# JuliaGenAI/ColBERT.jl

Measured on AMD Instinct MI355X. Metric: queries/sec, top-1000 on 1M-passage corpus, higher is better.
Workload: dtype f32

## Files before the change

colbert.jl_amd/csrc/approx_kernels.hpp:

```cpp
#pragma once
#include <hip/hip_fp16.h>

#include <algorithm>

#include "common.hpp"
#include "search_kernels.hpp"

namespace clb {

typedef __bf16 bf16x8 __attribute__((ext_vector_type(8)));
typedef uint32_t u32x4 __attribute__((ext_vector_type(4)));
typedef uint32_t u32x4_a4 __attribute__((ext_vector_type(4), aligned(4)));
typedef float f32x4_a4 __attribute__((ext_vector_type(4), aligned(4)));

constexpr float kEpsSafety = 1.25f;

inline bool approx_supported(int dim, int nbits) { return dim == kDim && nbits == 2; }
inline size_t approx_cells_bytes(int64_t B, int64_t K, int64_t ) { return (size_t)B * K * 16 * 4 + 2048; }

__device__ __forceinline__ uint32_t f32_to_bf16_rne(float f) {
    const uint32_t u = __float_as_uint(f);
    return (u + 0x7fffu + ((u >> 16) & 1u)) >> 16;
}
__device__ __forceinline__ uint32_t pack_bf16(float lo, float hi) {
// ... 739 lines not shown
        }
        const float v[4] = {__uint_as_float(lo.x), __uint_as_float(lo.z), __uint_as_float(hi.x), __uint_as_float(hi.z)};
        const int id[4] = {(int)lo.y, (int)lo.w, (int)hi.y, (int)hi.w};
#pragma unroll
        for (int e = 0; e < 4; ++e) {
            const bool take = id[e] != 0x7fffffff && v[e] >= thr;
            const unsigned long long m = __builtin_amdgcn_ballot_w64(take);
            if (m == 0) break;
            const int pos = total + __popcll(m & ((1ull << lane) - 1ull));
            if (take && pos < kTopRefineCap) cand[pos] = ValIdx{v[e], id[e]};
            total += __popcll(m);
        }
    }
    __syncthreads();
    const bool overflow = total > kTopRefineCap || last_max >= thr;
    float tv[2] = {kNegInf, kNegInf};
    int ti[2] = {0x7fffffff, 0x7fffffff};
    if (!overflow) {
        for (int g0 = 0; g0 < total; g0 += kTopRefine) {
        const int grp = g0 + (lane >> 4), rr = lane & 15;
        const int gid = grp < total ? cand[grp].i : 0;
        const int id = (gid >> 1) * 32 + (rr & 3) + 8 * (rr >> 2) + 4 * (gid & 1);
        if (grp < total && id < K) {
            const float4* c4 = reinterpret_cast<const float4*>(C + (size_t)id * kDim);
            float4 cr[32];
#pragma unroll
            for (int m = 0; m < 32; ++m) cr[m] = c4[m];
            float a = 0.f;
#pragma unroll
            for (int m = 0; m < 32; ++m) {
                a = fmaf(cr[m].x, qs[4 * m], a);
                a = fmaf(cr[m].y, qs[4 * m + 1], a);
                a = fmaf(cr[m].z, qs[4 * m + 2], a);
                a = fmaf(cr[m].w, qs[4 * m + 3], a);
            }
            topn_insert<2>(tv, ti, a, id);
        }
        }
    } else {
        for (int c = lane; c < K; c += 64) {
            const float* cr = C + (size_t)c * kDim;
            float a = 0.f;
            for (int d = 0; d < kDim; ++d) a = fmaf(cr[d], qs[d], a);
            topn_insert<2>(tv, ti, a, c);
        }
        if (lane == 0) atomicAdd(&redo_flag[b], 1);
    }
#pragma unroll
    for (int o = 32; o > 0; o >>= 1) {
        const float v0 = __shfl_xor(tv[0], o, 64), v1 = __shfl_xor(tv[1], o, 64);
        const int i0 = __shfl_xor(ti[0], o, 64), i1 = __shfl_xor(ti[1], o, 64);
        topn_insert<2>(tv, ti, v0, i0);
        topn_insert<2>(tv, ti, v1, i1);
    }
    if (lane == 0) {
        sel[((size_t)b * 32 + t) * 2] = ti[0];
        sel[((size_t)b * 32 + t) * 2 + 1] = ti[1] == 0x7fffffff ? ti[0] : ti[1];
    }
}

static __global__ __launch_bounds__(256) void cells_to_half_kernel(const float* __restrict__ cells,
                                                                  uint32_t* __restrict__ cells16, int K) {
    const int b = blockIdx.y;
    const float* src = cells + (size_t)b * K * 32;
    uint32_t* dst = cells16 + (size_t)b * K * 16;
    const int64_t total = (int64_t)K * 16;
    for (int64_t i = (int64_t)blockIdx.x * 256 + threadIdx.x; i < total; i += (int64_t)gridDim.x * 256) {
        const int64_t c = i >> 4;
        const int t = (int)(i & 15);
        const float lo = src[c * 32 + 2 * t], hi = src[c * 32 + 2 * t + 1];
        const __half2 h = __floats2half2_rn(lo, hi);
        dst[i] = *reinterpret_cast<const uint32_t*>(&h);
    }
}

typedef _Float16 f16x8 __attribute__((ext_vector_type(8)));
typedef float f32x2 __attribute__((ext_vector_type(2)));

struct StepTag {
    int j;
    int rows;
    int last;
    int base;
};

constexpr int kStepRows = 32;

__device__ __forceinline__ uint32_t f32_to_f16_floor(float x) {
    const __half hr = __float2half_rn(x);
    uint32_t bits = *reinterpret_cast<const uint16_t*>(&hr);
    if (__half2float(hr) > x) bits = (bits & 0x8000u) ? bits + 1u : (bits == 0u ? 0x8001u : bits - 1u);
    return bits;
}

template <int N>
__device__ __forceinline__ uint32_t lut_offset(uint32_t R, uint32_t lane8) {
    return __builtin_amdgcn_perm(R, lane8, 0x0c0c0000u | ((4u + N) << 8));
}

#define CLB_DPP_F(V, CTRL) __builtin_bit_cast(float, __builtin_amdgcn_update_dpp(0, __builtin_bit_cast(int, (V)), (CTRL), 0xf, 0xf, true))
__device__ __forceinline__ float sum_lanes_0_31(float s) {
    s += CLB_DPP_F(s, 0xB1);
    s += CLB_DPP_F(s, 0x4E);
    s += CLB_DPP_F(s, 0x141);
    s += CLB_DPP_F(s, 0x140);
    const float below = __builtin_bit_cast(float, __builtin_amdgcn_update_dpp(0, __builtin_bit_cast(int, s), 0x142, 0xa, 0xf, false));
    return s + below;
}
__device__ __forceinline__ float max_lane_halves(float m) { return fmaxf(m, __shfl_xor(m, 32, 64)); }

#ifndef CLB_APPROX_WAVES
#define CLB_APPROX_WAVES 12
#endif
#ifdef CLB_APPROX_SPLIT_LUT
constexpr bool kSplitLut = true;
#else
constexpr bool kSplitLut = false;
#endif
#if defined(CLB_APPROX_PRIO) && CLB_APPROX_PRIO
#define CLB_APPROX_PRIO_UP __builtin_amdgcn_s_setprio(CLB_APPROX_PRIO);
#define CLB_APPROX_PRIO_DOWN __builtin_amdgcn_s_setprio(0);
#else
#define CLB_APPROX_PRIO_UP
#define CLB_APPROX_PRIO_DOWN
#endif
#ifndef CLB_APPROX_MINOCC
#define CLB_APPROX_MINOCC (CLB_APPROX_WAVES / 4)
#endif
constexpr int kApproxThreads = 64 * CLB_APPROX_WAVES;
constexpr int kApproxLdsLut = 256 * 256;

template <bool ROWS, int ABL = 0, int GL = 0, int PIPE = 0, bool CELL8 = false>
static __global__ __launch_bounds__(kApproxThreads, CLB_APPROX_MINOCC) void score_approx32_kernel(
    const float* __restrict__ weights, const uint32_t* __restrict__ codeinv, const uint8_t* __restrict__ residuals,
    int cbits, float inv_lo, float inv_step, const float* __restrict__ Q, const uint32_t* __restrict__ cells16,
    const uint2* __restrict__ cand_hdr, const int* __restrict__ ncand, float* __restrict__ scores, int K, int T,
    int B, size_t cand_cap, uint16_t* __restrict__ tokmax, const int* __restrict__ list,
    const int* __restrict__ nlist, const float* __restrict__ eps_pair, unsigned long long* __restrict__ rowmask,
    const float4* __restrict__ tscale = nullptr) {
    const uint32_t cmask = (1u << cbits) - 1u;
    const int lane = threadIdx.x & 63;
    const int r = lane & 31, h = lane >> 5;
    const int x = blockIdx.x & 7;
    const int wg = blockIdx.x >> 3;
    const int wg_per_group = gridDim.x >> 3;
    const int wave = __builtin_amdgcn_readfirstlane(threadIdx.x >> 6);
    __shared__ __attribute__((aligned(16))) unsigned char lut_s[kApproxLdsLut];
    __shared__ __attribute__((aligned(16))) float invx[kApproxThreads / 64][2 * kStepRows];
    static_assert(GL == 0 || ABL == 0, "the ablation variants exist for the VGPR gather only");
    static_assert(!CELL8 || ABL == 0, "the ablation variants exist for the fp16 score rows only");
    constexpr int kSlotBytes = CELL8 ? 1024 : 2048;
    constexpr int kRingBytes = 3 * kSlotBytes;
    static_assert(GL == 0 || CLB_APPROX_WAVES <= 12, "the 3-slot ring of the LDS-DMA form fits 160 KB of LDS up to 12 waves");
    __shared__ __attribute__((aligned(16))) unsigned char ring_s[GL ? (kApproxThreads / 64) * kRingBytes : 16];
    constexpr int kStageBytes = 16 * 64 + 64;
    __shared__ __attribute__((aligned(16))) unsigned char stage_s[ROWS ? 16 : (kApproxThreads / 64) * kStageBytes];
    unsigned char* mystage = stage_s + (ROWS ? 0 : wave * kStageBytes);
    for (int i = threadIdx.x; i < 256 * 32; i += kApproxThreads) {
        const int v = i >> 5;
        *reinterpret_cast<uint2*>(lut_s + (size_t)i * 8) =
            make_uint2(pack_f16(weights[v & 3], weights[(v >> 2) & 3]), pack_f16(weights[(v >> 4) & 3], weights[(v >> 6) & 3]));
    }
    __syncthreads();
    const char* lut = reinterpret_cast<const char*>(lut_s);
    float* myinv = invx[wave];
    const uint32_t lane8 = 8u * (uint32_t)r;
    unsigned char* myring = ring_s + (GL ? wave * kRingBytes : 0);
    const uint32_t ring_lds = (uint32_t)(uintptr_t)(__attribute__((address_space(3))) unsigned char*)myring;
    const uint32_t gl_poff = 16u * (((uint32_t)lane - (((uint32_t)lane >> 4) & 3u)) & 3u);
    const int gl_src0 = (int)((uint32_t)lane & ~3u);
    const int gl_src1 = gl_src0 + 64;
    const uint32_t gl_rot = ((uint32_t)r >> 2) & 3u;
    const uint32_t gl_x0 = (uint32_t)r * 64u + 16u * (((uint32_t)h + gl_rot) & 3u);
    const uint32_t gl_x1 = (uint32_t)r * 64u + 16u * (((uint32_t)h + 2u + gl_rot) & 3u);
    const int gl8_src = (int)(((uint32_t)lane >> 1) << 2);
    const uint32_t gl8_poff = 16u * (((uint32_t)lane ^ ((uint32_t)lane >> 4)) & 1u);
    const uint32_t gl8_x = (uint32_t)r * 32u + 16u * (((uint32_t)h ^ ((uint32_t)r >> 3)) & 1u);

    f16x8 sel1, sel2;
#pragma unroll
    for (int j = 0; j < 8; ++j) {
        sel1[j] = (r == (CELL8 ? 16 * h + j : 8 * h + j)) ? (_Float16)1.0f : (_Float16)0.0f;
        sel2[j] = (r == (CELL8 ? 16 * h + 8 + j : 16 + 8 * h + j)) ? (_Float16)1.0f : (_Float16)0.0f;
    }

    int b_first, b_step, sub, nsub;
    if (B >= 8) { b_first = x; b_step = 8; sub = 0; nsub = 1; }
    else { b_first = x % B; b_step = B * 8 ; sub = x / B; nsub = (8 - b_first + B - 1) / B; }
    const bool grid2d = gridDim.y > 1;
    const int wg_count = grid2d ? (int)gridDim.x : wg_per_group;
    const int wg_index = grid2d ? (int)blockIdx.x : wg;
    if (grid2d) { b_first = blockIdx.y; b_step = B; sub = 0; nsub = 1; }

    for (int b = b_first; b < B; b += b_step) {
        u32x4 qb[8];
        const float4 ts = CELL8 ? tscale[(size_t)b * 32 + r] : make_float4(1.f, 1.f, 0.f, 0.f);
        const float stp = ts.x;
        const float acc_init = CELL8 ? ts.z - 1024.0f : 0.f;
        {
            const float* qrow = Q + ((size_t)b * T + (r < T ? r : T - 1)) * kDim + 64 * h;
#pragma unroll
            for (int s = 0; s < 8; ++s) {
                float4 lo = *reinterpret_cast<const float4*>(qrow + 8 * s);
                float4 hi = *reinterpret_cast<const float4*>(qrow + 8 * s + 4);
                if (r >= T) { lo = make_float4(0.f, 0.f, 0.f, 0.f); hi = lo; }
                if (CELL8) {
                    lo.x *= ts.y; lo.y *= ts.y; lo.z *= ts.y; lo.w *= ts.y;
                    hi.x *= ts.y; hi.y *= ts.y; hi.z *= ts.y; hi.w *= ts.y;
                }
                qb[s] = u32x4{pack_f16(lo.x, lo.y), pack_f16(lo.z, lo.w), pack_f16(hi.x, hi.y), pack_f16(hi.z, hi.w)};
            }
        }
        const uint2* hdr = cand_hdr + (size_t)b * cand_cap;
        const char* c16 = reinterpret_cast<const char*>(cells16 + (size_t)b * K * (CELL8 ? 8 : 16));
        const uint32_t h16 = 16u * (uint32_t)h;
        float* out = scores + (size_t)b * cand_cap;
        uint16_t* tmax = tokmax + (size_t)b * cand_cap * 32 + r;
        const int* lst = ROWS ? list + (size_t)b * cand_cap : nullptr;
        unsigned long long* rmask = ROWS ? rowmask + (size_t)b * cand_cap * 4 : nullptr;
        const float window = ROWS ? 2.f * eps_pair[b] : 0.f;
        const int n = ROWS ? nlist[b] : ncand[b];
        const int n_waves = wg_count * (kApproxThreads / 64) * nsub;
        const int my_wave = (sub * wg_count + wg_index) * (kApproxThreads / 64) + wave;
        const int per_wave = (n + n_waves - 1) / n_waves;
        const int j_first = min(n, my_wave * per_wave), j_end = min(n, j_first + per_wave);
        unsigned long long wm0 = 0, wm1 = 0, wm2 = 0, wm3 = 0;

        for (int j0 = j_first; j0 < j_end; j0 += 64) {
        const int jl = j0 + lane;
        int slot_l = jl < j_end ? jl : j0;
        if (ROWS) slot_l = lst[slot_l];
        const uint2 hv = hdr[slot_l];
        const int nd = j_end - j0 < 64 ? j_end - j0 : 64;
        int it_k = 0;
        uint32_t it_off = __builtin_amdgcn_readlane(hv.x, 0);
        int it_len = (int)__builtin_amdgcn_readlane(hv.y, 0);
        int it_slot = __builtin_amdgcn_readlane(slot_l, 0);
        int it_base = 0;
        const uint32_t abl_stride = ABL == 11 ? ((uint32_t)__builtin_amdgcn_readlane(hv.x, nd - 1) - it_off) / (uint32_t)nd : 0u;
        if (ABL == 11) it_len = 82;
        const uint32_t abl_bound = ABL == 11 ? (uint32_t)__builtin_amdgcn_readlane(hv.x, nd - 1) : 0u;

#define CLB_STAGE_A(RB, CV, PM, TAG)                                                                    \
    {                                                                                                       \
        const bool live = it_k < nd;                                                                        \
        const uint32_t e0 = live ? (ABL == 11 ? min(it_off + (uint32_t)it_base, abl_bound) : it_off + (uint32_t)it_base) : 0u; \
        const int left = live ? it_len - it_base : kStepRows;                                               \
        const int rows = left < kStepRows ? left : kStepRows;                                               \
        if (ROWS) PM = tmax[(size_t)(live ? it_slot : 0) * 32];    \
        const uint32_t rr = min((uint32_t)r, (uint32_t)(rows - 1));    \
         \
        const uint8_t* rbase_ = residuals + (size_t)e0 * 32;                                                \
        const uint32_t* cbase_ = codeinv + (size_t)e0;                                                      \
        const uint32_t roff_ = rr * 32u + h16;                                                              \
         \
         \
        if (ABL == 3 || ABL == 7) RB = u32x4{e0 * 2654435761u + rr, e0 ^ h16, e0 + 77u * rr, e0 * 40503u};  \
        else if (ABL == 4) RB = *reinterpret_cast<const u32x4*>(rbase_ + roff_);                            \
        else RB = __builtin_nontemporal_load(reinterpret_cast<const u32x4*>(rbase_ + roff_));               \
        if (ABL == 7) CV = (e0 * 97u + rr) & 131071u;                                                       \
        else if (ABL == 4) CV = cbase_[rr];                                                                 \
        else CV = __builtin_nontemporal_load(cbase_ + rr);                    \
        TAG.j = live ? j0 + it_k : -1;                                                                      \
        TAG.rows = rows;                                                                                    \
        TAG.last = left <= kStepRows ? (it_k + 1 >= nd ? 3 : 1) : 0;                                        \
        TAG.base = it_base;                                                                                 \
        it_base += kStepRows;                                                                               \
        if (ABL == 11) {         \
            if (TAG.last) { it_k += 1; it_off += abl_stride; it_base = 0; }                                 \
        } else                                                                                              \
        if (TAG.last) {                                                                                     \
            it_k += 1;                                                                                      \
            const int kk = it_k < 64 ? it_k : 63;                                                           \
            it_off = __builtin_amdgcn_readlane(hv.x, kk);                                                   \
            it_len = (int)__builtin_amdgcn_readlane(hv.y, kk);                                              \
            it_slot = __builtin_amdgcn_readlane(slot_l, kk);                                                \
            it_base = 0;                                                                                    \
        }                                                                                                   \
    }
#define CLB_STAGE_G(CV, X0, X1, SLOT)                                                                       \
    if (GL && CELL8) {                                                                                      \
        const uint32_t ca_ = (uint32_t)__builtin_amdgcn_ds_bpermute(gl8_src, (int)CV) & cmask;              \
        asm volatile("s_mov_b32 m0, %1\n\tglobal_load_lds_dwordx4 %0, off"                                  \
                     :: "v"(c16 + ((ca_ << 5) + gl8_poff)), "s"(ring_lds + (SLOT) * 1024u) : "memory");     \
    } else if (GL) {                                                                                        \
        const uint32_t ca_ = (uint32_t)__builtin_amdgcn_ds_bpermute(gl_src0, (int)CV) & cmask;              \
        const uint32_t cb_ = (uint32_t)__builtin_amdgcn_ds_bpermute(gl_src1, (int)CV) & cmask;              \
         \
        asm volatile("s_mov_b32 m0, %2\n\tglobal_load_lds_dwordx4 %0, off\n\t"                            \
                     "s_add_u32 m0, m0, 0x400\n\tglobal_load_lds_dwordx4 %1, off"                          \
                     :: "v"(c16 + ((ca_ << 6) + gl_poff)), "v"(c16 + ((cb_ << 6) + gl_poff)),               \
                        "s"(ring_lds + (SLOT) * 2048u) : "memory", "scc");                                   \
    } else {                                                                                                \
        const char* row_ = CELL8 ? c16 + (((CV & cmask) << 5) + h16)                                        \
                                 : c16 + (((ABL == 2 ? (CV & 1023u) : (CV & cmask)) << 6) + h16);           \
        if (ABL == 1 || ABL == 7) { X0 = u32x4{CV, CV, CV, CV}; X1 = X0; }                                  \
        else if (CELL8) X0 = *reinterpret_cast<const u32x4*>(row_);       \
        else {                                                                                              \
        X0 = *reinterpret_cast<const u32x4*>(row_);                                                         \
        X1 = *reinterpret_cast<const u32x4*>(row_ + 32);                                                    \
        }                                                                                                   \
    }
#define CLB_LUT(W, N) (*reinterpret_cast<const uint2*>(lut + lut_offset<N>(W, lane8)))
#define CLB_STAGE_CM(RB, CV, X0, X1, SLOT, ACC, INVB)                                                       \
    {                                                                                                       \
        if (GL && CELL8) {                                                                                  \
             \
            asm volatile("s_waitcnt vmcnt(3)" ::: "memory");                                                \
            X0 = *reinterpret_cast<const u32x4*>(myring + (SLOT) * 1024 + gl8_x);                           \
        } else if (GL) {                                                                                    \
             \
            asm volatile("s_waitcnt vmcnt(4)" ::: "memory");                                                \
            X0 = *reinterpret_cast<const u32x4*>(myring + (SLOT) * 2048 + gl_x0);                           \
            X1 = *reinterpret_cast<const u32x4*>(myring + (SLOT) * 2048 + gl_x1);                           \
        }                                                                                                   \
         \
        __builtin_amdgcn_wave_barrier();                                                                    \
        myinv[(INVB) * kStepRows + r] = fmaf((float)(CV >> cbits), inv_step, inv_lo);                                            \
        __builtin_amdgcn_wave_barrier();                                                                    \
         \
         \
         \
        uint2 tl[16];                                                                                       \
        if (ABL != 5) {                                                                                     \
            tl[0] = CLB_LUT(RB[0], 0); tl[1] = CLB_LUT(RB[0], 1); tl[2] = CLB_LUT(RB[0], 2); tl[3] = CLB_LUT(RB[0], 3);     \
            tl[4] = CLB_LUT(RB[1], 0); tl[5] = CLB_LUT(RB[1], 1); tl[6] = CLB_LUT(RB[1], 2); tl[7] = CLB_LUT(RB[1], 3);     \
            if (!kSplitLut) {                                                                               \
            tl[8] = CLB_LUT(RB[2], 0); tl[9] = CLB_LUT(RB[2], 1); tl[10] = CLB_LUT(RB[2], 2); tl[11] = CLB_LUT(RB[2], 3);   \
            tl[12] = CLB_LUT(RB[3], 0); tl[13] = CLB_LUT(RB[3], 1); tl[14] = CLB_LUT(RB[3], 2); tl[15] = CLB_LUT(RB[3], 3); \
            }                                                                                               \
        }                                                                                                   \
        __builtin_amdgcn_sched_barrier(0);                                                                  \
        CLB_APPROX_PRIO_UP                                                                                  \
        _Pragma("unroll") for (int i = 0; i < 16; ++i) ACC[i] = acc_init;                                   \
        if (CELL8) {                     \
            const u32x4 raw_ = X0;                                                                          \
            X0 = u32x4{__builtin_amdgcn_perm(0x64646464u, raw_[0], 0x04010400u), __builtin_amdgcn_perm(0x64646464u, raw_[0], 0x04030402u), \
                       __builtin_amdgcn_perm(0x64646464u, raw_[1], 0x04010400u), __builtin_amdgcn_perm(0x64646464u, raw_[1], 0x04030402u)}; \
            X1 = u32x4{__builtin_amdgcn_perm(0x64646464u, raw_[2], 0x04010400u), __builtin_amdgcn_perm(0x64646464u, raw_[2], 0x04030402u), \
                       __builtin_amdgcn_perm(0x64646464u, raw_[3], 0x04010400u), __builtin_amdgcn_perm(0x64646464u, raw_[3], 0x04030402u)}; \
        }                                                                                                   \
        ACC = __builtin_amdgcn_mfma_f32_32x32x16_f16(__builtin_bit_cast(f16x8, X0), sel1, ACC, 0, 0, 0);    \
        ACC = __builtin_amdgcn_mfma_f32_32x32x16_f16(__builtin_bit_cast(f16x8, X1), sel2, ACC, 0, 0, 0);    \
        if (ABL == 5) { ACC[0] += __uint_as_float(RB[0] ^ RB[1]); ACC[1] += __uint_as_float(RB[2] ^ RB[3]); } \
        else {                                                                                              \
            _Pragma("unroll") for (int s_ = 0; s_ < 8; ++s_) {                                              \
                if (kSplitLut && s_ == 4) {       \
                    __builtin_amdgcn_sched_barrier(0);                                                      \
                    tl[0] = CLB_LUT(RB[2], 0); tl[1] = CLB_LUT(RB[2], 1); tl[2] = CLB_LUT(RB[2], 2); tl[3] = CLB_LUT(RB[2], 3);   \
                    tl[4] = CLB_LUT(RB[3], 0); tl[5] = CLB_LUT(RB[3], 1); tl[6] = CLB_LUT(RB[3], 2); tl[7] = CLB_LUT(RB[3], 3);   \
                    __builtin_amdgcn_sched_barrier(0);                                                      \
                }                                                                                           \
                const int ti_ = kSplitLut ? 2 * (s_ & 3) : 2 * s_;                                          \
                ACC = __builtin_amdgcn_mfma_f32_32x32x16_f16(                                               \
                    __builtin_bit_cast(f16x8, u32x4{tl[ti_].x, tl[ti_].y, tl[ti_ + 1].x, tl[ti_ + 1].y}),   \
                    __builtin_bit_cast(f16x8, qb[s_]), ACC, 0, 0, 0);                                       \
            }                                                                                               \
        }                                                                                                   \
        CLB_APPROX_PRIO_DOWN                                                                                \
    }
#define CLB_STAGE_E(ACC, INVB, PM, TAG)                                                                     \
    {                                                                                                       \
        f32x4 iq[4];                                                                                        \
        _Pragma("unroll") for (int q = 0; q < 4; ++q)                                                       \
            iq[q] = *reinterpret_cast<const f32x4*>(myinv + (INVB) * kStepRows + 8 * q + 4 * h);                                 \
         \
         \
         \
        float v[16];                                                                                        \
        if (ABL != 6) { _Pragma("unroll") for (int i = 0; i < 16; ++i) { v[i] = ACC[i] * iq[i >> 2][i & 3]; asm volatile("" : "+v"(v[i])); } } \
        else                                                                                                \
        _Pragma("unroll") for (int i = 0; i < 16; i += 2) {     \
            const f32x2 p_ = f32x2{ACC[i], ACC[i + 1]} * f32x2{iq[i >> 2][i & 3], iq[i >> 2][(i & 3) + 1]}; \
            v[i] = p_[0]; v[i + 1] = p_[1];                                                                 \
        }                                                                                                   \
        if (ROWS) {                                                                                         \
            const __half pmh = *reinterpret_cast<const __half*>(&PM);                                       \
            const float lo = r < T ? __half2float(pmh) - window : __builtin_inff();    \
             \
             \
             \
            uint32_t lm = 0;                                                                                \
            _Pragma("unroll") for (int i = 0; i < 16; ++i) lm |= !((CELL8 ? v[i] * stp : v[i]) < lo) ? (1u << i) : 0u; \
            lm |= (uint32_t)__builtin_amdgcn_update_dpp(0, (int)lm, 0xB1, 0xf, 0xf, true);         \
            lm |= (uint32_t)__builtin_amdgcn_update_dpp(0, (int)lm, 0x4E, 0xf, 0xf, true);         \
            lm |= (uint32_t)__builtin_amdgcn_update_dpp(0, (int)lm, 0x141, 0xf, 0xf, true);    \
            lm |= (uint32_t)__builtin_amdgcn_update_dpp(0, (int)lm, 0x140, 0xf, 0xf, true);      \
            const uint32_t m0_ = __builtin_amdgcn_readlane(lm, 0) | __builtin_amdgcn_readlane(lm, 16);      \
            const uint32_t m1_ = __builtin_amdgcn_readlane(lm, 32) | __builtin_amdgcn_readlane(lm, 48);     \
             \
            uint32_t bits = ((m0_ & 0xFu) | ((m0_ & 0xF0u) << 4) | ((m0_ & 0xF00u) << 8) | ((m0_ & 0xF000u) << 12)) | \
                            (((m1_ & 0xFu) | ((m1_ & 0xF0u) << 4) | ((m1_ & 0xF00u) << 8) | ((m1_ & 0xF000u) << 12)) << 4); \
            if (TAG.rows < kStepRows) bits &= (1u << TAG.rows) - 1u;        \
            const unsigned long long wbits = (unsigned long long)bits << (TAG.base & 32);                   \
            const int wi = TAG.base >> 6;                                                                   \
            wm0 |= wi == 0 ? wbits : 0ull;                                                                  \
            wm1 |= wi == 1 ? wbits : 0ull;                                                                  \
            wm2 |= wi == 2 ? wbits : 0ull;                                                                  \
            wm3 |= wi == 3 ? wbits : 0ull;                                                                  \
            if (TAG.last) {                                                                                 \
                if (lane == 0 && TAG.j >= 0) {                                                              \
                    unsigned long long* o = rmask + (size_t)TAG.j * 4;                                      \
                    o[0] = wm0; o[1] = wm1; o[2] = wm2; o[3] = wm3;                                         \
                }                                                                                           \
                wm0 = wm1 = wm2 = wm3 = 0;                                                                  \
            }                                                                                               \
        } else {                                                                                            \
            float m01 = fmaxf(fmaxf(v[0], v[1]), v[2]);                                                     \
            float m23 = fmaxf(fmaxf(v[3], v[4]), v[5]);                                                     \
            float m45 = fmaxf(fmaxf(v[6], v[7]), v[8]);                                                     \
            float m67 = fmaxf(fmaxf(v[9], v[10]), v[11]);                                                   \
            float m89 = fmaxf(fmaxf(v[12], v[13]), v[14]);                                                  \
            m01 = fmaxf(fmaxf(m01, m23), m45);                                                              \
            m67 = fmaxf(fmaxf(m67, m89), v[15]);                                                            \
            mx = fmaxf(fmaxf(mx, m01), m67);                                                                \
            if (ABL == 10) {      \
                const float lo = r < T ? mx - 0.09f : __builtin_inff();                                     \
                uint32_t lm = 0;                                                                            \
                _Pragma("unroll") for (int i = 0; i < 16; ++i) lm |= !(v[i] < lo) ? (1u << i) : 0u;         \
                lm |= (uint32_t)__builtin_amdgcn_update_dpp(0, (int)lm, 0xB1, 0xf, 0xf, true);              \
                lm |= (uint32_t)__builtin_amdgcn_update_dpp(0, (int)lm, 0x4E, 0xf, 0xf, true);              \
                lm |= (uint32_t)__builtin_amdgcn_update_dpp(0, (int)lm, 0x141, 0xf, 0xf, true);             \
                lm |= (uint32_t)__builtin_amdgcn_update_dpp(0, (int)lm, 0x140, 0xf, 0xf, true);             \
                const uint32_t m0_ = __builtin_amdgcn_readlane(lm, 0) | __builtin_amdgcn_readlane(lm, 16);  \
                const uint32_t m1_ = __builtin_amdgcn_readlane(lm, 32) | __builtin_amdgcn_readlane(lm, 48); \
                uint32_t bits = ((m0_ & 0xFu) | ((m0_ & 0xF0u) << 4) | ((m0_ & 0xF00u) << 8) | ((m0_ & 0xF000u) << 12)) | \
                                (((m1_ & 0xFu) | ((m1_ & 0xF0u) << 4) | ((m1_ & 0xF00u) << 8) | ((m1_ & 0xF000u) << 12)) << 4); \
                if (TAG.rows < kStepRows) bits &= (1u << TAG.rows) - 1u;                                    \
                const unsigned long long wbits = (unsigned long long)bits << (TAG.base & 32);               \
                const int wi = TAG.base >> 6;                                                               \
                wm0 |= wi == 0 ? wbits : 0ull; wm1 |= wi == 1 ? wbits : 0ull;                               \
                wm2 |= wi == 2 ? wbits : 0ull; wm3 |= wi == 3 ? wbits : 0ull;                               \
            }                                                                                               \
            if (TAG.last) {                                                                                 \
                if (ABL == 10) {      \
                    if (lane == 0 && TAG.j >= 0) {                                                          \
                        unsigned long long* o = rowmask + ((size_t)b * cand_cap + TAG.j) * 4;               \
                        o[0] = wm0; o[1] = wm1; o[2] = wm2; o[3] = wm3;                                     \
                    }                                                                                       \
                    wm0 = wm1 = wm2 = wm3 = 0;                                                              \
                }                                                                                           \
                mx = max_lane_halves(mx);                                                                   \
                if (CELL8) mx *= stp;                    \
                const float sum = sum_lanes_0_31(r < T ? mx : 0.f);              \
                if (ABL == 8) { if (sum == 12345.678f) out[0] = mx; }         \
                else if (TAG.j >= 0) {                                                                      \
                     \
                    const int p_ = (TAG.j - j0) & 15;                                                       \
                    if (h == 0) *reinterpret_cast<uint16_t*>(mystage + p_ * 64 + 2 * r) = (uint16_t)f32_to_f16_floor(mx); \
                    if (lane == 16) *reinterpret_cast<float*>(mystage + 1024 + 4 * p_) = sum;               \
                    if (p_ == 15 || TAG.last == 3) {     \
                        const int jb_ = TAG.j - p_;                                                         \
                        __builtin_amdgcn_wave_barrier();                                                    \
                        const u32x4 tk_ = *reinterpret_cast<const u32x4*>(mystage + 16 * lane);             \
                        const float sc_ = *reinterpret_cast<const float*>(mystage + 1024 + 4 * (lane & 15)); \
                        if (lane < 4 * (p_ + 1))                                                            \
                            *reinterpret_cast<u32x4*>(reinterpret_cast<unsigned char*>(tokmax + ((size_t)b * cand_cap + jb_) * 32) + 16 * lane) = tk_; \
                        if (lane <= p_) out[jb_ + lane] = sc_;                                              \
                        __builtin_amdgcn_wave_barrier();                                                    \
                    }                                                                                       \
                }                                                                                           \
                mx = kNegInf;                                                                               \
            }                                                                                               \
        }                                                                                                   \
    }

        float mx = kNegInf;
        u32x4 rb0, rb1, rb2, xa0, xa1, xa2, xb0, xb1, xb2;
        uint32_t cv0, cv1, cv2, cw0, cw1, cw2;
        uint16_t pm0 = 0, pm1 = 0, pm2 = 0;
        StepTag t0, t1, t2;
        f32x16 acc0, acc1;
        CLB_STAGE_A(rb0, cv0, pm0, t0);
        CLB_STAGE_A(rb1, cv1, pm1, t1);
        CLB_STAGE_G(cv0, xa0, xb0, 0); cw0 = cv0;
        if (!PIPE) {
            while (t0.j >= 0) {
                CLB_STAGE_A(rb2, cv2, pm2, t2);
                CLB_STAGE_G(cv1, xa1, xb1, 1); cw1 = cv1;
                CLB_STAGE_CM(rb0, cw0, xa0, xb0, 0, acc0, 0);
                CLB_STAGE_E(acc0, 0, pm0, t0);
                CLB_STAGE_A(rb0, cv0, pm0, t0);
                CLB_STAGE_G(cv2, xa2, xb2, 2); cw2 = cv2;
                CLB_STAGE_CM(rb1, cw1, xa1, xb1, 1, acc0, 0);
                CLB_STAGE_E(acc0, 0, pm1, t1);
                CLB_STAGE_A(rb1, cv1, pm1, t1);
                CLB_STAGE_G(cv0, xa0, xb0, 0); cw0 = cv0;
                CLB_STAGE_CM(rb2, cw2, xa2, xb2, 2, acc0, 0);
                CLB_STAGE_E(acc0, 0, pm2, t2);
            }
        } else {
            StepTag tp; tp.j = -1; tp.rows = kStepRows; tp.last = 1; tp.base = 0;
            uint16_t pmp = 0;
#pragma unroll
            for (int i = 0; i < 16; ++i) { acc0[i] = 0.f; acc1[i] = 0.f; }
            for (;;) {
                if (t0.j < 0) { CLB_STAGE_E(acc1, 1, pmp, tp); break; }
                CLB_STAGE_A(rb2, cv2, pm2, t2);
                CLB_STAGE_G(cv1, xa1, xb1, 1); cw1 = cv1;
                CLB_STAGE_CM(rb0, cw0, xa0, xb0, 0, acc0, 0);
                CLB_STAGE_E(acc1, 1, pmp, tp);
                tp = t0; pmp = pm0;
                CLB_STAGE_A(rb0, cv0, pm0, t0);
                CLB_STAGE_G(cv2, xa2, xb2, 2); cw2 = cv2;
                CLB_STAGE_CM(rb1, cw1, xa1, xb1, 1, acc1, 1);
                CLB_STAGE_E(acc0, 0, pmp, tp);
                tp = t1; pmp = pm1;
                CLB_STAGE_A(rb1, cv1, pm1, t1);
                CLB_STAGE_G(cv0, xa0, xb0, 0); cw0 = cv0;
                CLB_STAGE_CM(rb2, cw2, xa2, xb2, 2, acc0, 0);
                CLB_STAGE_E(acc1, 1, pmp, tp);
                tp = t2; pmp = pm2;
                if (t0.j < 0) { CLB_STAGE_E(acc0, 0, pmp, tp); break; }
                CLB_STAGE_A(rb2, cv2, pm2, t2);
                CLB_STAGE_G(cv1, xa1, xb1, 1); cw1 = cv1;
                CLB_STAGE_CM(rb0, cw0, xa0, xb0, 0, acc1, 1);
                CLB_STAGE_E(acc0, 0, pmp, tp);
                tp = t0; pmp = pm0;
                CLB_STAGE_A(rb0, cv0, pm0, t0);
                CLB_STAGE_G(cv2, xa2, xb2, 2); cw2 = cv2;
                CLB_STAGE_CM(rb1, cw1, xa1, xb1, 1, acc0, 0);
                CLB_STAGE_E(acc1, 1, pmp, tp);
                tp = t1; pmp = pm1;
                CLB_STAGE_A(rb1, cv1, pm1, t1);
                CLB_STAGE_G(cv0, xa0, xb0, 0); cw0 = cv0;
                CLB_STAGE_CM(rb2, cw2, xa2, xb2, 2, acc1, 1);
                CLB_STAGE_E(acc0, 0, pmp, tp);
                tp = t2; pmp = pm2;
            }
        }
        }
#undef CLB_STAGE_A
#undef CLB_STAGE_G
#undef CLB_STAGE_CM
#undef CLB_STAGE_E
#undef CLB_LUT
    }
}

static __global__ __launch_bounds__(256) void code_adjacency_kernel(const uint32_t* __restrict__ codes0, int64_t n,
                                                                   unsigned long long* __restrict__ count) {
    unsigned long long c = 0;
    for (int64_t i = (int64_t)blockIdx.x * 256 + threadIdx.x + 1; i < n; i += (int64_t)gridDim.x * 256)
        c += (codes0[i] >> 1) == (codes0[i - 1] >> 1);
#pragma unroll
    for (int o = 32; o > 0; o >>= 1) c += __shfl_xor(c, o, 64);
    if ((threadIdx.x & 63) == 0 && c) atomicAdd(count, c);
}

struct ApproxConsts {
    float cn_max;
    float rn_max;
    float inv_max;
    float rb_max;
    float dw_rn;
    float inv_qerr;
    float dc_max;
};

struct QueryBound { float eps_t, eps_sum; bool unsafe; };
__device__ __forceinline__ QueryBound query_bound(const float* __restrict__ Q, int b, int T, const ApproxConsts& ac,
                                                  float* s_qn, float* s_dq, const float4* __restrict__ tscale = nullptr,
                                                  float* s_aux = nullptr ,
                                                  bool cell8 = false) {
    const int tid = threadIdx.x;
    if (tid == 0) { *s_qn = 0.f; *s_dq = 0.f; }
    if (tscale && tid < 4) s_aux[tid] = 0.f;
    __syncthreads();
    {
        const int t = tid >> 5, part = tid & 31;
        float a = 0.f, dd = 0.f, d8 = 0.f;
        if (t < T) {
            const float4 v = *reinterpret_cast<const float4*>(Q + ((size_t)b * T + t) * kDim + 4 * part);
            a = fmaf(v.x, v.x, fmaf(v.y, v.y, fmaf(v.z, v.z, v.w * v.w)));
            const float dx = v.x - round_f16(v.x), dy = v.y - round_f16(v.y);
            const float dz = v.z - round_f16(v.z), dw = v.w - round_f16(v.w);
            dd = fmaf(dx, dx, fmaf(dy, dy, fmaf(dz, dz, dw * dw)));
            if (tscale && cell8) {
                const float4 ts = tscale[(size_t)b * 32 + t];
                const float sx = v.x * ts.y, sy = v.y * ts.y, sz = v.z * ts.y, sw = v.w * ts.y;
                const float ex = sx - round_f16(sx), ey = sy - round_f16(sy), ez = sz - round_f16(sz), ew = sw - round_f16(sw);
                d8 = fmaf(ex, ex, fmaf(ey, ey, fmaf(ez, ez, ew * ew)));
            }
        }
#pragma unroll
        for (int o = 16; o > 0; o >>= 1) { a += __shfl_xor(a, o, 64); dd += __shfl_xor(dd, o, 64); d8 += __shfl_xor(d8, o, 64); }
        if (t < T && part == 0) {
            atomicMax(reinterpret_cast<unsigned int*>(s_qn), __float_as_uint(sqrtf(a) * 1.001f));
            atomicMax(reinterpret_cast<unsigned int*>(s_dq), __float_as_uint(sqrtf(dd) * 1.001f));
            if (tscale) {
                const float4 ts = tscale[(size_t)b * 32 + t];
                atomicMax(reinterpret_cast<unsigned int*>(s_aux), __float_as_uint(ts.x * sqrtf(d8) * 1.001f));
                atomicMax(reinterpret_cast<unsigned int*>(s_aux + 1), __float_as_uint(ts.x));
                atomicMax(reinterpret_cast<unsigned int*>(s_aux + 3), __float_as_uint(ts.w));
                if (!(ts.x > 0.f) || !(sqrtf(a) * ts.y < 3.0e4f)) s_aux[2] = 1.f;
            }
        }
    }
    __syncthreads();
    const float u = 5.9604645e-08f;
    const float qn = *s_qn;
    const float e_cells = kEpsSafety * centroid_product_bound(qn, *s_dq, ac.cn_max, ac.dc_max) + 4.8828125e-04f * qn * ac.cn_max + 2.9802322e-08f;
    float e_qr = 1.001f * (*s_dq * ac.rb_max + qn * ac.dw_rn) + 2.f * 128.f * u * qn * ac.rn_max;
    float e_tab = e_cells;
    bool bad8 = false;
    if (tscale) {
        const float amax = s_aux[2] != 0.f ? qn * ac.cn_max : fminf(s_aux[3] * 1.0001f, qn * ac.cn_max);
        const float e_f16 = kEpsSafety * centroid_product_bound(qn, *s_dq, ac.cn_max, ac.dc_max) + 4.8828125e-04f * amax + 2.9802322e-08f;
        e_tab = e_f16;
        if (cell8) {
            const float dq8 = s_aux[0], step_max = s_aux[1];
            e_tab = e_f16 + 0.5005f * step_max + 8.f * u * amax;
            e_qr = 1.001f * ((dq8 + 2.f * u * qn) * ac.rb_max + qn * ac.dw_rn) +
                   2.f * 130.f * u * (amax + 255.f * step_max + qn * ac.rn_max) + 1280.f * u * step_max;
            bad8 = s_aux[2] != 0.f;
        }
    }
    const float eps_t = (ac.inv_max + ac.inv_qerr) * (e_tab + e_qr) + 1.01f * ac.inv_qerr * qn * (ac.cn_max + ac.rn_max) + 332.f * u * qn;
// ... 527 lines not shown
```

colbert.jl_amd/csrc/search.hip:

```cpp
#include <algorithm>
#include <cstdlib>
#include <cstring>
#include <numeric>

#include "approx_kernels.hpp"
#include "generic_kernels.hpp"
#include "search_kernels.hpp"
#include "sort.hpp"

using namespace clb;

namespace {

enum KernelId {
    KID_CENTROID_SCORES = 0,
    KID_TOPN,
    KID_MARK,
    KID_COMPACT,
    KID_SCORE_EXACT,
    KID_SCORE_APPROX,
    KID_SELECT,
    KID_ROWS,
    KID_TOPK,
    KID_COUNT
// ... 560 lines not shown
    CLB_HIP(hipMemsetAsync(w.wsel.p, 0, sizeof(WideSel) * B, st));
    const dim3 grid(kWideBlocks, B);
    ApproxConsts acw = s->approx_consts;
    acw.dc_max = bound_dc(s, w);
    hipLaunchKernelGGL(wide_minmax_kernel, grid, dim3(1024), 0, st, w.scores.as<float>(), w.ncand.as<int>(), dQ, T, w.cand_cap,
                       acw, w.wsel.as<WideSel>(), w.eps_pair.as<float>(),
                       w.have_range ? (const float4*)w.tscale.as<float4>() : (const float4*)nullptr, w.cell8 ? 1 : 0);
    if (!tau_in)
        for (int pass = 0; pass < 4; ++pass)
            hipLaunchKernelGGL(wide_hist_kernel, grid, dim3(1024), 0, st, w.scores.as<float>(), w.ncand.as<int>(), k, w.cand_cap,
                               w.wsel.as<WideSel>(), pass);
    hipLaunchKernelGGL(wide_count_kernel, grid, dim3(1024), 0, st, w.scores.as<float>(), w.ncand.as<int>(), k, w.cand_cap,
                       w.wsel.as<WideSel>(), tau_in);
    hipLaunchKernelGGL(wide_emit_kernel, grid, dim3(1024), 0, st, w.scores.as<float>(), w.ncand.as<int>(), k, w.cand_cap,
                       (const WideSel*)w.wsel.as<WideSel>(), tau_in, w.list.as<int>(), w.nlist.as<int>(), w.thresh.as<float>());
    return CLB_OK;
}

int run_search(clb_searcher* s, Workspace& w, hipStream_t st, const float* dQ, int B, int T, int nprobe, int k,
               int64_t* d_out_pids, float* d_out_scores, int64_t* d_n_cand = nullptr, int phase = 0,
               float* d_local_top = nullptr, const float* d_all_top = nullptr, int n_shards = 0) {
    if (s->generic || T > 128) {
        if (phase != 0) return fail(CLB_EUNSUPPORTED, "the two-phase sharded search needs the two-pass mode");
        return run_search_general(s, w, st, dQ, B, T, nprobe, k, d_out_pids, d_out_scores, d_n_cand);
    }
    const int kpow2 = next_pow2(std::min(k, (int)kMaxTopK));
    const int* list = nullptr;
    const int* nlist = nullptr;
    s->prof.chain = nullptr;
    const bool two_pass = s->mode == 1 && s->approx_ok && T <= 32;
    if (phase != 0 && !two_pass) return fail(CLB_EUNSUPPORTED, "the two-phase sharded search needs the two-pass mode");
    if (phase == 2) {
        CLB_TRY(w.tau_glob.ensure(sizeof(float) * B));
        hipLaunchKernelGGL(global_tau_kernel, dim3(B), dim3(1024), 0, st, d_all_top, n_shards, B, k,
                           w.tau_glob.as<float>());
        Timed t(s, KID_SELECT, st);
        CLB_TRY(launch_select(s, w, st, dQ, B, T, k, (const float*)w.tau_glob.as<float>()));
        list = w.list.as<int>();
        nlist = w.nlist.as<int>();
    }
    if (phase != 2) {
    CLB_TRY(run_retrieve(s, w, st, dQ, B, T, nprobe));
    if (s->prof.counters) {
        if (!w.stats_keep) CLB_HIP(hipMemsetAsync(w.stats.p, 0, sizeof(unsigned long long) * 8, st));
        s->prof.chain = nullptr;
    }
    if (two_pass) {
        {
            Timed t(s, KID_SCORE_APPROX, st);
            const int wgpg = CLB_KNOB("CLB_DEBUG_APPROX_WGPG", 32);
            const int approx_2d = CLB_KNOB("CLB_DEBUG_APPROX_2D", -1);
            const double est_cand = 0.5 * T * nprobe * (double)s->n_emb / (double)std::max<int64_t>(1, s->K);
            int gxq = est_cand < 6000.0 ? std::max(8, 256 / B) : 0;
            if (approx_2d >= 0) gxq = approx_2d > 0 ? std::max(1, approx_2d / B) : 0;
            const dim3 approx_grid = gxq > 0 && B > 1 ? dim3(gxq, B) : dim3(8 * wgpg);
#define CLB_LAUNCH_APPROX(ABL)                                                                                        \
    hipLaunchKernelGGL((score_approx32_kernel<false, ABL>), approx_grid, dim3(kApproxThreads), 0, st, s->weights.as<float>(), \
                       s->codeinv.as<uint32_t>(), s->residuals.as<uint8_t>(), s->cbits, s->inv_lo, s->inv_step, dQ,  \
                       w.cells_q.as<uint32_t>(), w.cand_hdr.as<uint2>(), w.ncand.as<int>(), w.scores.as<float>(), \
                       (int)s->K, T, B, w.cand_cap, w.tokmax.as<uint16_t>(), (const int*)nullptr,                    \
                       (const int*)nullptr, (const float*)nullptr, (unsigned long long*)nullptr)
#ifdef CLB_ABLATIONS
            if (CLB_KNOB("CLB_DEBUG_APPROX_PIPE", 0)) {
#if CLB_APPROX_WAVES <= 12
                auto kern = s->gather_lds ? score_approx32_kernel<false, 0, 1, 1> : score_approx32_kernel<false, 0, 0, 1>;
#else
                auto kern = score_approx32_kernel<false, 0, 0, 1>;
#endif
                hipLaunchKernelGGL(kern, approx_grid, dim3(kApproxThreads), 0, st, s->weights.as<float>(),
                                   s->codeinv.as<uint32_t>(), s->residuals.as<uint8_t>(), s->cbits, s->inv_lo, s->inv_step, dQ,
                                   w.cells_q.as<uint32_t>(), w.cand_hdr.as<uint2>(), w.ncand.as<int>(), w.scores.as<float>(),
                                   (int)s->K, T, B, w.cand_cap, w.tokmax.as<uint16_t>(), (const int*)nullptr,
                                   (const int*)nullptr, (const float*)nullptr, (unsigned long long*)nullptr, (const float4*)nullptr);
            } else
            switch (CLB_KNOB("CLB_DEBUG_APPROX_VARIANT", 0)) {
                case 1: CLB_LAUNCH_APPROX(1); break;
                case 2: CLB_LAUNCH_APPROX(2); break;
                case 3: CLB_LAUNCH_APPROX(3); break;
                case 4: CLB_LAUNCH_APPROX(4); break;
                case 5: CLB_LAUNCH_APPROX(5); break;
                case 6: CLB_LAUNCH_APPROX(6); break;
                case 7: CLB_LAUNCH_APPROX(7); break;
                case 8: CLB_LAUNCH_APPROX(8); break;
                case 11: CLB_LAUNCH_APPROX(11); break;
                case 10:
                    hipLaunchKernelGGL((score_approx32_kernel<false, 10>), approx_grid, dim3(kApproxThreads), 0, st, s->weights.as<float>(),
                                       s->codeinv.as<uint32_t>(), s->residuals.as<uint8_t>(), s->cbits, s->inv_lo, s->inv_step, dQ,
                                       w.cells_q.as<uint32_t>(), w.cand_hdr.as<uint2>(), w.ncand.as<int>(), w.scores.as<float>(),
                                       (int)s->K, T, B, w.cand_cap, w.tokmax.as<uint16_t>(), (const int*)nullptr,
                                       (const int*)nullptr, (const float*)nullptr, w.rowmask.as<unsigned long long>());
                    break;
                default: launch_pass1(s, w, st, dQ, approx_grid, B, T);
            }
#else
            launch_pass1(s, w, st, dQ, approx_grid, B, T);
#endif
#undef CLB_LAUNCH_APPROX
        }
        {
            Timed t(s, KID_SELECT, st);
            CLB_TRY(launch_select(s, w, st, dQ, B, T, k, nullptr, phase == 0));
        }
        list = w.list.as<int>();
        nlist = w.nlist.as<int>();
    }
    }
    if (phase == 1) {
        hipLaunchKernelGGL(local_top_kernel, dim3(B), dim3(1024), 0, st, w.scores.as<float>(), list, nlist,
                           w.thresh.as<float>(), k, w.cand_cap, d_local_top);
        CLB_HIP(hipGetLastError());
        return CLB_OK;
    }
    const bool subset = list && !CLB_KNOB("CLB_DEBUG_NO_SUBSET", 0);
    if (subset) {
        Timed t(s, KID_ROWS, st);
        const int rows_gx = CLB_KNOB("CLB_DEBUG_ROWS_GX", 256);
        const dim3 rows_grid = B > 1 ? dim3(std::max(1, rows_gx / B), B) : dim3(8 * 32);
        auto rows_kernel = w.cell8 ? score_approx32_kernel<true, 0, 0, 0, true> : score_approx32_kernel<true, 0, 0, 0, false>;
        hipLaunchKernelGGL(rows_kernel, rows_grid, dim3(kApproxThreads), 0, st, s->weights.as<float>(),
                           s->codeinv.as<uint32_t>(), s->residuals.as<uint8_t>(), s->cbits, s->inv_lo, s->inv_step, dQ,
                           w.cell8 ? w.cells8.as<uint32_t>() : w.cells_q.as<uint32_t>(), w.cand_hdr.as<uint2>(), w.ncand.as<int>(),
                           w.scores.as<float>(), (int)s->K, T, B, w.cand_cap, w.tokmax.as<uint16_t>(), list, nlist,
                           w.eps_pair.as<float>(), w.rowmask.as<unsigned long long>(), (const float4*)w.tscale.as<float4>());
    }
    {
        Timed t(s, KID_SCORE_EXACT, st);
        const int gxl = CLB_KNOB("CLB_DEBUG_EXACT_GX", 1024);
        const int gx = list ? std::max(1, gxl / B) : std::max(1, 2048 / B);
        const int flat_gx = CLB_KNOB("CLB_DEBUG_FLAT_GX", 768);
        if (subset) {
            hipLaunchKernelGGL(score_exact_flat_kernel, dim3(std::max(1, flat_gx / B), B), dim3(256), 0, st, s->centroids.as<float>(),
                               s->weights.as<float>(), s->codes0.as<uint32_t>(), s->residuals.as<uint8_t>(),
                               w.cand_hdr.as<uint2>(), dQ, w.scores.as<float>(), T, w.cand_cap, list, nlist,
                               w.rowmask.as<unsigned long long>());
        } else
        switch (s->nbits) {
            case 1: launch_score_exact<1>(s, w, st, dQ, B, T, list, nlist, gx); break;
            case 2: launch_score_exact<2>(s, w, st, dQ, B, T, list, nlist, gx); break;
            case 4: launch_score_exact<4>(s, w, st, dQ, B, T, list, nlist, gx); break;
            default: return fail(CLB_EUNSUPPORTED, "nbits=%d not supported by the HIP search path", s->nbits);
        }
    }
    if (k <= kMaxTopK) {
        Timed t(s, KID_TOPK, st);
        allow_large_topk_lds();
        const int ranked = list != nullptr && !CLB_KNOB("CLB_DEBUG_NO_RANK", 0);
        if (ranked)
            hipLaunchKernelGGL(topk_rank_kernel, dim3(kRankBlocks, B), dim3(1024), 0, st, w.scores.as<float>(),
                               w.cand.as<uint32_t>(), w.ncand.as<int>(), list, nlist, k, w.cand_cap, s->pid_offset,
                               d_out_pids, d_out_scores, w.flags.as<int>(), d_n_cand);
        hipLaunchKernelGGL(topk_kernel, dim3(B), dim3(1024), sizeof(unsigned long long) * kpow2, st,
                           w.scores.as<float>(), w.cand.as<uint32_t>(), w.ncand.as<int>(), list, nlist, k,
                           kpow2, w.cand_cap, s->pid_offset, d_out_pids, d_out_scores, w.flags.as<int>(), d_n_cand, ranked);
    } else {
        s->prof.chain = nullptr;
        for (int b = 0; b < B; ++b) CLB_TRY(topk_by_sort(s, w, st, b, list, nlist, k, d_out_pids, d_out_scores, d_n_cand));
    }
    if (s->prof.counters) {
        hipLaunchKernelGGL(batch_stats_kernel, dim3(32, B), dim3(256), 0, st, w.cand.as<uint32_t>(),
                           w.ncand.as<int>(), list, nlist, s->doc_off.as<uint32_t>(), w.cand_cap,
                           w.stats.as<unsigned long long>(),
                           subset ? w.rowmask.as<unsigned long long>() : (const unsigned long long*)nullptr);
    }
    CLB_HIP(hipGetLastError());
    return CLB_OK;
}

// ... 586 lines not shown
```

Measured before the change: 29050.

## Pack the tail of one passage with the next passage into a shared 32-row step

```diff
diff --git a/colbert.jl_amd/csrc/approx_kernels.hpp b/colbert.jl_amd/csrc/approx_kernels.hpp
--- a/colbert.jl_amd/csrc/approx_kernels.hpp
+++ b/colbert.jl_amd/csrc/approx_kernels.hpp
@@ -845,9 +845,14 @@
     int rows;
     int last;
     int base;
+    int g;
+    int jh;
+    int rowsh;
+    int baseh;
 };
 
 constexpr int kStepRows = 32;
+constexpr uint32_t kPackSpan = (1u << 27) - kStepRows;
 
 __device__ __forceinline__ uint32_t f32_to_f16_floor(float x) {
     const __half hr = __float2half_rn(x);
@@ -917,6 +922,7 @@
     static_assert(GL == 0 || CLB_APPROX_WAVES <= 12, "the 3-slot ring of the LDS-DMA form fits 160 KB of LDS up to 12 waves");
     __shared__ __attribute__((aligned(16))) unsigned char ring_s[GL ? (kApproxThreads / 64) * kRingBytes : 16];
     constexpr int kStageBytes = 16 * 64 + 64;
+    constexpr bool kPack = !ROWS && ABL != 10;
     __shared__ __attribute__((aligned(16))) unsigned char stage_s[ROWS ? 16 : (kApproxThreads / 64) * kStageBytes];
     unsigned char* mystage = stage_s + (ROWS ? 0 : wave * kStageBytes);
     for (int i = threadIdx.x; i < 256 * 32; i += kApproxThreads) {
@@ -1000,46 +1006,68 @@
         int it_len = (int)__builtin_amdgcn_readlane(hv.y, 0);
         int it_slot = __builtin_amdgcn_readlane(slot_l, 0);
         int it_base = 0;
-        const uint32_t abl_stride = ABL == 11 ? ((uint32_t)__builtin_amdgcn_readlane(hv.x, nd - 1) - it_off) / (uint32_t)nd : 0u;
-        if (ABL == 11) it_len = 82;
-        const uint32_t abl_bound = ABL == 11 ? (uint32_t)__builtin_amdgcn_readlane(hv.x, nd - 1) : 0u;
 
 #define CLB_STAGE_A(RB, CV, PM, TAG)                                                                    \
     {                                                                                                       \
         const bool live = it_k < nd;                                                                        \
-        const uint32_t e0 = live ? (ABL == 11 ? min(it_off + (uint32_t)it_base, abl_bound) : it_off + (uint32_t)it_base) : 0u; \
+        const uint32_t e0 = live ? it_off + (uint32_t)it_base : 0u;                                         \
         const int left = live ? it_len - it_base : kStepRows;                                               \
         const int rows = left < kStepRows ? left : kStepRows;                                               \
-        if (ROWS) PM = tmax[(size_t)(live ? it_slot : 0) * 32];    \
-        const uint32_t rr = min((uint32_t)r, (uint32_t)(rows - 1));    \
+        int slot_t = live ? it_slot : 0;                                                                    \
+        uint32_t d_ = 0;                                                                                    \
+        TAG.j = live ? j0 + it_k : -1;                                                                      \
+        TAG.rows = rows;                                                                                    \
+        TAG.last = 0;                                                                                       \
+        TAG.base = it_base;                                                                                 \
+        TAG.g = 0; TAG.jh = -1; TAG.rowsh = rows; TAG.baseh = 0;                                            \
+        if (left <= kStepRows) {                                        \
+            const int kb = it_k + 1;                                                                        \
+            const int kk = kb < 64 ? kb : 63;                                                               \
+            const uint32_t off_b = __builtin_amdgcn_readlane(hv.x, kk);                                     \
+            const int len_b = (int)__builtin_amdgcn_readlane(hv.y, kk);                                     \
+            const int slot_b = __builtin_amdgcn_readlane(slot_l, kk);                                       \
+            const int gq = (rows + 7) >> 3;                                                                 \
+            d_ = off_b - e0;                     \
+            if (kPack && gq >= 1 && gq < 4 && kb < nd && len_b > 0 && d_ < kPackSpan) {    \
+                const int cap = kStepRows - 8 * gq;                                                         \
+                TAG.g = gq; TAG.jh = TAG.j; TAG.rowsh = rows; TAG.baseh = it_base;                          \
+                TAG.j = j0 + kb; TAG.rows = len_b < cap ? len_b : cap; TAG.base = 0;                         \
+                slot_t = slot_b;                                                                            \
+                if (len_b <= cap) {                                           \
+                    TAG.last = kb + 1 >= nd ? 3 : 1;                                                        \
+                    it_k = kb + 1;                                                                          \
+                    const int kc = it_k < 64 ? it_k : 63;                                                   \
+                    it_off = __builtin_amdgcn_readlane(hv.x, kc);                                           \
+                    it_len = (int)__builtin_amdgcn_readlane(hv.y, kc);                                      \
+                    it_slot = __builtin_amdgcn_readlane(slot_l, kc);                                        \
+                    it_base = 0;                                                                            \
+                } else {                                                                                    \
+                    it_k = kb; it_off = off_b; it_len = len_b; it_slot = slot_b; it_base = cap;             \
+                }                                                                                           \
+            } else {                                                                                        \
+                d_ = 0;                                                                                     \
+                TAG.last = kb >= nd ? 3 : 1;                                                                \
+                it_k = kb; it_off = off_b; it_len = len_b; it_slot = slot_b; it_base = 0;                   \
+            }                                                                                               \
+        } else it_base += kStepRows;                                                                        \
+        if (ROWS) PM = tmax[(size_t)slot_t * 32];               \
+        const uint32_t q8_ = 8u * (uint32_t)TAG.g;                                                          \
+                       \
+        const uint32_t rr = (uint32_t)r < q8_ ? min((uint32_t)r, (uint32_t)(TAG.rowsh - 1))                 \
+                                              : min((uint32_t)r, q8_ + (uint32_t)(TAG.rows - 1)) + (d_ - q8_); \
          \
         const uint8_t* rbase_ = residuals + (size_t)e0 * 32;                                                \
-        const uint32_t* cbase_ = codeinv + (size_t)e0;                                                      \
+        const char* cbase_ = reinterpret_cast<const char*>(codeinv + (size_t)e0);                           \
         const uint32_t roff_ = rr * 32u + h16;                                                              \
+        const uint32_t coff_ = rr * 4u;                                                                     \
          \
          \
         if (ABL == 3 || ABL == 7) RB = u32x4{e0 * 2654435761u + rr, e0 ^ h16, e0 + 77u * rr, e0 * 40503u};  \
         else if (ABL == 4) RB = *reinterpret_cast<const u32x4*>(rbase_ + roff_);                            \
         else RB = __builtin_nontemporal_load(reinterpret_cast<const u32x4*>(rbase_ + roff_));               \
         if (ABL == 7) CV = (e0 * 97u + rr) & 131071u;                                                       \
-        else if (ABL == 4) CV = cbase_[rr];                                                                 \
-        else CV = __builtin_nontemporal_load(cbase_ + rr);                    \
-        TAG.j = live ? j0 + it_k : -1;                                                                      \
-        TAG.rows = rows;                                                                                    \
-        TAG.last = left <= kStepRows ? (it_k + 1 >= nd ? 3 : 1) : 0;                                        \
-        TAG.base = it_base;                                                                                 \
-        it_base += kStepRows;                                                                               \
-        if (ABL == 11) {         \
-            if (TAG.last) { it_k += 1; it_off += abl_stride; it_base = 0; }                                 \
-        } else                                                                                              \
-        if (TAG.last) {                                                                                     \
-            it_k += 1;                                                                                      \
-            const int kk = it_k < 64 ? it_k : 63;                                                           \
-            it_off = __builtin_amdgcn_readlane(hv.x, kk);                                                   \
-            it_len = (int)__builtin_amdgcn_readlane(hv.y, kk);                                              \
-            it_slot = __builtin_amdgcn_readlane(slot_l, kk);                                                \
-            it_base = 0;                                                                                    \
-        }                                                                                                   \
+        else if (ABL == 4) CV = *reinterpret_cast<const uint32_t*>(cbase_ + coff_);                         \
+        else CV = __builtin_nontemporal_load(reinterpret_cast<const uint32_t*>(cbase_ + coff_));    \
     }
 #define CLB_STAGE_G(CV, X0, X1, SLOT)                                                                       \
     if (GL && CELL8) {                                                                                      \
@@ -1122,6 +1150,29 @@
         }                                                                                                   \
         CLB_APPROX_PRIO_DOWN                                                                                \
     }
+#define CLB_PASSAGE_END(MX, J, LAST)                                                                        \
+    {                                                                                                       \
+        float m_ = max_lane_halves(MX);                                                                     \
+        if (CELL8) m_ *= stp;                         \
+        const float sum = sum_lanes_0_31(r < T ? m_ : 0.f);                      \
+        if (ABL == 8) { if (sum == 12345.678f) out[0] = m_; }                \
+        else if ((J) >= 0) {                                                                                \
+                   \
+            const int p_ = ((J) - j0) & 15;                                                                 \
+            if (h == 0) *reinterpret_cast<uint16_t*>(mystage + p_ * 64 + 2 * r) = (uint16_t)f32_to_f16_floor(m_); \
+            if (lane == 16) *reinterpret_cast<float*>(mystage + 1024 + 4 * p_) = sum;                       \
+            if (p_ == 15 || (LAST) == 3) {     \
+                const int jb_ = (J) - p_;                                                                   \
+                __builtin_amdgcn_wave_barrier();                                                            \
+                const u32x4 tk_ = *reinterpret_cast<const u32x4*>(mystage + 16 * lane);                     \
+                const float sc_ = *reinterpret_cast<const float*>(mystage + 1024 + 4 * (lane & 15));         \
+                if (lane < 4 * (p_ + 1))                                                                    \
+                    *reinterpret_cast<u32x4*>(reinterpret_cast<unsigned char*>(tokmax + ((size_t)b * cand_cap + jb_) * 32) + 16 * lane) = tk_; \
+                if (lane <= p_) out[jb_ + lane] = sc_;                                                      \
+                __builtin_amdgcn_wave_barrier();                                                            \
+            }                                                                                               \
+        }                                                                                                   \
+    }
 #define CLB_STAGE_E(ACC, INVB, PM, TAG)                                                                     \
     {                                                                                                       \
         f32x4 iq[4];                                                                                        \
@@ -1169,6 +1220,15 @@
                 wm0 = wm1 = wm2 = wm3 = 0;                                                                  \
             }                                                                                               \
         } else {                                                                                            \
+            if (TAG.g) {               \
+                const float q0_ = fmaxf(fmaxf(fmaxf(v[0], v[1]), v[2]), v[3]);                              \
+                const float q1_ = fmaxf(fmaxf(fmaxf(v[4], v[5]), v[6]), v[7]);                              \
+                const float q2_ = fmaxf(fmaxf(fmaxf(v[8], v[9]), v[10]), v[11]);                            \
+                const float q3_ = fmaxf(fmaxf(fmaxf(v[12], v[13]), v[14]), v[15]);                          \
+                const float mh_ = fmaxf(fmaxf(mx, q0_), fmaxf(TAG.g > 1 ? q1_ : kNegInf, TAG.g > 2 ? q2_ : kNegInf)); \
+                CLB_PASSAGE_END(mh_, TAG.jh, 1);                                                            \
+                mx = fmaxf(fmaxf(TAG.g > 1 ? kNegInf : q1_, TAG.g > 2 ? kNegInf : q2_), q3_);               \
+            } else {                                                                                        \
             float m01 = fmaxf(fmaxf(v[0], v[1]), v[2]);                                                     \
             float m23 = fmaxf(fmaxf(v[3], v[4]), v[5]);                                                     \
             float m45 = fmaxf(fmaxf(v[6], v[7]), v[8]);                                                     \
@@ -1177,6 +1237,7 @@
             m01 = fmaxf(fmaxf(m01, m23), m45);                                                              \
             m67 = fmaxf(fmaxf(m67, m89), v[15]);                                                            \
             mx = fmaxf(fmaxf(mx, m01), m67);                                                                \
+            }                                                                                               \
             if (ABL == 10) {      \
                 const float lo = r < T ? mx - 0.09f : __builtin_inff();                                     \
                 uint32_t lm = 0;                                                                            \
@@ -1203,26 +1264,7 @@
                     }                                                                                       \
                     wm0 = wm1 = wm2 = wm3 = 0;                                                              \
                 }                                                                                           \
-                mx = max_lane_halves(mx);                                                                   \
-                if (CELL8) mx *= stp;                    \
-                const float sum = sum_lanes_0_31(r < T ? mx : 0.f);              \
-                if (ABL == 8) { if (sum == 12345.678f) out[0] = mx; }         \
-                else if (TAG.j >= 0) {                                                                      \
-                     \
-                    const int p_ = (TAG.j - j0) & 15;                                                       \
-                    if (h == 0) *reinterpret_cast<uint16_t*>(mystage + p_ * 64 + 2 * r) = (uint16_t)f32_to_f16_floor(mx); \
-                    if (lane == 16) *reinterpret_cast<float*>(mystage + 1024 + 4 * p_) = sum;               \
-                    if (p_ == 15 || TAG.last == 3) {     \
-                        const int jb_ = TAG.j - p_;                                                         \
-                        __builtin_amdgcn_wave_barrier();                                                    \
-                        const u32x4 tk_ = *reinterpret_cast<const u32x4*>(mystage + 16 * lane);             \
-                        const float sc_ = *reinterpret_cast<const float*>(mystage + 1024 + 4 * (lane & 15)); \
-                        if (lane < 4 * (p_ + 1))                                                            \
-                            *reinterpret_cast<u32x4*>(reinterpret_cast<unsigned char*>(tokmax + ((size_t)b * cand_cap + jb_) * 32) + 16 * lane) = tk_; \
-                        if (lane <= p_) out[jb_ + lane] = sc_;                                              \
-                        __builtin_amdgcn_wave_barrier();                                                    \
-                    }                                                                                       \
-                }                                                                                           \
+                CLB_PASSAGE_END(mx, TAG.j, TAG.last);                                                       \
                 mx = kNegInf;                                                                               \
             }                                                                                               \
         }                                                                                                   \
@@ -1254,6 +1296,7 @@
             }
         } else {
             StepTag tp; tp.j = -1; tp.rows = kStepRows; tp.last = 1; tp.base = 0;
+            tp.g = 0; tp.jh = -1; tp.rowsh = kStepRows; tp.baseh = 0;
             uint16_t pmp = 0;
 #pragma unroll
             for (int i = 0; i < 16; ++i) { acc0[i] = 0.f; acc1[i] = 0.f; }
@@ -1297,6 +1340,7 @@
 #undef CLB_STAGE_G
 #undef CLB_STAGE_CM
 #undef CLB_STAGE_E
+#undef CLB_PASSAGE_END
 #undef CLB_LUT
     }
 }
diff --git a/colbert.jl_amd/csrc/search.hip b/colbert.jl_amd/csrc/search.hip
--- a/colbert.jl_amd/csrc/search.hip
+++ b/colbert.jl_amd/csrc/search.hip
@@ -666,7 +666,6 @@
                 case 6: CLB_LAUNCH_APPROX(6); break;
                 case 7: CLB_LAUNCH_APPROX(7); break;
                 case 8: CLB_LAUNCH_APPROX(8); break;
-                case 11: CLB_LAUNCH_APPROX(11); break;
                 case 10:
                     hipLaunchKernelGGL((score_approx32_kernel<false, 10>), approx_grid, dim3(kApproxThreads), 0, st, s->weights.as<float>(),
                                        s->codeinv.as<uint32_t>(), s->residuals.as<uint8_t>(), s->cbits, s->inv_lo, s->inv_step, dQ,
```

Result: faster. 29720 (median of 6 runs) (+2.3%).
